# soldasim/BOSS.jl

Hardware: AMD Instinct MI355X
Metric: gp_posterior_updates_per_sec (+ acq_evals_per_sec), N=4096 d=8 fp64 (higher is better)
Workload: dtype f64; 1 GPU; d=8 synthetic blackbox, GaussianProcess(Matern52) surrogate, N=4096 fp64 posterior update + ExpectedImprovement over 8192 candidates per GPU (BASELINE.json configs[1]+[2]); N=4096, d=8, M_per_gpu=8192, kernel=matern52, parallelism=single GPU: no exchange

## Files before the change

### boss.jl_amd/csrc/bosship.hip

```cpp
#include "../../include/bosship.h"

#include <hip/hip_runtime.h>

#include <algorithm>
#include <cmath>
#include <cstdint>
#include <cstdio>
#include <cstdlib>
#include <atomic>
#include <chrono>
#include <cstring>
#include <functional>
#include <limits>
#include <map>
#include <mutex>
#include <string>
#include <thread>
#include <vector>

#include "gp_kernels.hpp"
#include "potrf.hpp"
#include "chain.hpp"
#include "small_calls.hpp"
#include "rider.hpp"
// ... 42 lines not shown
}

constexpr size_t MULTI_RES_OFF = 384;
constexpr size_t FEW_RES_OFF = 400;

struct Workspace {
    void* p = nullptr;
    size_t bytes = 0;
};

struct Ctx {
    int device = -1;
    int logical = -1;
    hipStream_t own_stream = nullptr;
    hipStream_t stream = nullptr;
    hipStream_t side_stream = nullptr;
    std::vector<hipEvent_t> ev_panel, ev_rest;
    hipEvent_t ev_fork = nullptr, ev_up = nullptr;
    unsigned long long* sig_panel = nullptr;
    unsigned long long* sig_panel_host = nullptr;
    unsigned long long sig_seq = 0;
    hipStream_t chain_stream = nullptr, strip_stream = nullptr;
    unsigned long long chain_seq = 0, crit_seq = 0, up_seq = 0;
    int n_cus = 256;
    bool chain_ok = false;
    bool test_drop_chain = false;
    unsigned long long acq_seq = 0;
    unsigned long long few_seq = 0;
    std::mutex slab_mtx;
    void* slab_cache = nullptr;
    size_t slab_cache_bytes = 0;
    void* hostblk_cache = nullptr;
    size_t hostblk_cache_bytes = 0;
    unsigned long long* few_done = nullptr;
    unsigned long long few_done_cnt = 0;
    bool lookahead = true;
    bool prof_on = false;
    std::map<std::string, std::vector<std::pair<hipEvent_t, hipEvent_t>>> prof;
    std::vector<hipEvent_t> ev_pool;
    Workspace vscratch, csc, pred, acq, batchA, batchX, batchMisc, craw, lgA, lgB, lgC, few, setdesc, setmom;
    static constexpr int LLG_BANKS = 4;
    Workspace lgbank[LLG_BANKS - 1][3];
    hipStream_t llg_stream[LLG_BANKS - 1] = {nullptr, nullptr, nullptr};
    hipEvent_t llg_join[LLG_BANKS - 1] = {nullptr, nullptr, nullptr};
    void* pinned = nullptr;
    struct TrailTab {
        TrailWork* dev = nullptr;
        std::vector<TrailWork> host;
        std::vector<int> off;
    };
    TrailTab trail[65];
    std::mutex mtx;
};

static void chain_quiesce(Ctx* c) {
    if (c->chain_stream) (void)hipStreamSynchronize(c->chain_stream);
    if (c->strip_stream) (void)hipStreamSynchronize(c->strip_stream);
}

static std::mutex g_ctx_mtx;
static std::map<int, Ctx*> g_ctx;

static bool release_cached_slabs() {
    int dev = -1;
    if (hipGetDevice(&dev) != hipSuccess) return false;
    std::vector<void*> blocks;
// ... 5 lines not shown
            std::lock_guard<std::mutex> sl(c->slab_mtx);
            if (c->slab_cache) blocks.push_back(c->slab_cache);
            c->slab_cache = nullptr;
            c->slab_cache_bytes = 0;
        }
    }
    for (void* b : blocks) (void)hipFree(b);
    return !blocks.empty();
}
extern "C" int boss_debug_fail_next_alloc(int n) {
    g_fail_allocs.store(n > 0 ? n : 0);
    return BOSS_OK;
}
extern "C" int boss_debug_slab_cache_bytes(int device, size_t* bytes_out) {
    std::lock_guard<std::mutex> lk(g_ctx_mtx);
    auto it = g_ctx.find(device);
    if (bytes_out) *bytes_out = 0;
    if (it != g_ctx.end() && bytes_out) {
        std::lock_guard<std::mutex> sl(it->second->slab_mtx);
        *bytes_out = it->second->slab_cache_bytes;
    }
    return BOSS_OK;
}

static void ctx_destroy(Ctx* c) {
    if (!c) return;
    if (c->own_stream) (void)hipStreamDestroy(c->own_stream);
    if (c->side_stream) (void)hipStreamDestroy(c->side_stream);
    if (c->chain_stream) (void)hipStreamDestroy(c->chain_stream);
    if (c->strip_stream) (void)hipStreamDestroy(c->strip_stream);
    if (c->ev_fork) (void)hipEventDestroy(c->ev_fork);
    if (c->sig_panel && !c->sig_panel_host) (void)hipFree(c->sig_panel);
    if (c->few_done) (void)hipFree(c->few_done);
    for (auto& t : c->trail)
        if (t.dev) (void)hipFree(t.dev);
    if (c->slab_cache) (void)hipFree(c->slab_cache);
    if (c->hostblk_cache) (void)hipHostFree(c->hostblk_cache);
    if (c->ev_up) (void)hipEventDestroy(c->ev_up);
    for (int i = 0; i < Ctx::LLG_BANKS - 1; ++i) {
        if (c->llg_stream[i]) (void)hipStreamDestroy(c->llg_stream[i]);
        if (c->llg_join[i]) (void)hipEventDestroy(c->llg_join[i]);
    }
    if (c->pinned) (void)hipHostFree(c->pinned);
    delete c;
}

static int ctx_init(Ctx* c) {
    {
        int least = 0, greatest = 0;
        (void)hipDeviceGetStreamPriorityRange(&least, &greatest);
        static const int cu_mask = getenv("BOSS_CU_MASK") ? atoi(getenv("BOSS_CU_MASK")) : 0;
        if (cu_mask) {
            hipDeviceProp_t prop;
            HIPCHK(hipGetDeviceProperties(&prop, c->device));
            const int ncu = prop.multiProcessorCount, words = (ncu + 31) / 32;
            auto make = [&](hipStream_t* st, int lo, int hi) {
                std::vector<uint32_t> m(words, 0u);
                for (int b = lo; b < hi && b < ncu; ++b) m[b / 32] |= 1u << (b % 32);
                return hipExtStreamCreateWithCUMask(st, (uint32_t)words, m.data());
            };
            HIPCHK(make(&c->chain_stream, 0, 16));
            HIPCHK(make(&c->strip_stream, 16, 32));
            HIPCHK(make(&c->own_stream, 32, ncu));
            HIPCHK(make(&c->side_stream, cu_mask >= 2 ? 40 : 32, cu_mask >= 2 ? ncu : ncu - 8));
            c->stream = c->own_stream;
            std::fprintf(stderr, "[bosship] BOSS_CU_MASK=%d: chain on CU bits 0-15, strips on 16-31, main stream on 32-%d, side stream %d-%d\n",
// ... 241 lines not shown
    bool gated = false;
    bool chained = false;
    bool fell_back = false;
    int trail_used = -1;
    double* host_res = nullptr;
    double* host_res_dev = nullptr;
    bool par_in_args = false;
    unsigned long long res_seq = 0;
    bool res_polled = false;
    double* host_par = nullptr;
    hipEvent_t par_ev = nullptr;
    unsigned long long epoch = 0;
    unsigned long long factor_gen = 0, dinv0_gen = ~0ull;
    hipEvent_t dinv_ev = nullptr;
    bool dinv_pending = false;
    bool aug = false;
    int npts = 0, ldx = 0;
    bool gibbs = false;
    double *lamX = nullptr, *ampX = nullptr, *noiseX = nullptr;
    double *Winv = nullptr, *Linv = nullptr;
    double* W2 = nullptr;
    int w2_np = 0;
    unsigned long long w2_gen = ~0ull;
    bool w2_used = false;
    bool have_winv = false;
    int few_calls = 0;
    int append_calls = 0;
};

struct boss_cand {
    Ctx* ctx = nullptr;
    int d = 0, M = 0, Mp = 0;
    double* Craw = nullptr;
};

struct boss_track {
    Ctx* ctx = nullptr;
    boss_gp* gp = nullptr;
    int d = 0, M = 0, Mp = 0, tiles = 0, Ncap = 0, N = 0;
    unsigned long long epoch = 0;
    double *V = nullptr, *Csc = nullptr, *mu = nullptr, *var = nullptr, *mean = nullptr;
    bool has_mean = false;
};

static inline int round_up(int x, int m) { return (x + m - 1) / m * m; }
struct SetBatch {
    int nb = 1;
    size_t sA = 0, sInv16 = 0, sDinv = 0, sDinv2 = 0, sW = 0, sX = 0;
};
static void linv_enqueue(boss_gp* g, hipStream_t s, double* U, double* Lw, const SetBatch& B = SetBatch());
constexpr int MAX_ROWS = 46080;

extern "C" const char* boss_version(void) { return "bosship 0.1.0 (gfx950, fp64 MFMA)"; }
extern "C" const char* boss_last_error(void) { return g_last_error.c_str(); }

extern "C" int boss_device_count(int* n_out) {
    const int n = visible_devices();
    hipError_t e = n > 0 ? hipSuccess : hipErrorNoDevice;
    if (e != hipSuccess || n <= 0) {
        if (n_out) *n_out = 0;
        return fail(BOSS_E_NO_DEVICE, "no HIP device visible (bosship has no CPU fallback)");
    }
    if (n_out) *n_out = n;
    return BOSS_OK;
}

extern "C" int boss_set_stream(int device, void* hip_stream) {
    Ctx* c;
    int rc = get_ctx(device, &c);
    if (rc) return rc;
    std::lock_guard<std::mutex> lk(c->mtx);
    HIPCHK(hipStreamSynchronize(c->stream));
    c->stream = hip_stream ? (hipStream_t)hip_stream : c->own_stream;
    return BOSS_OK;
}

extern "C" int boss_device_sync(int device) {
    Ctx* c;
    int rc = get_ctx(device, &c);
    if (rc) return rc;
    HIPCHK(hipStreamSynchronize(c->stream));
    return BOSS_OK;
}

static bool few_done_ensure(Ctx* c, hipStream_t s) {
    if (c->few_done) return true;
    if (hipMalloc((void**)&c->few_done, sizeof(unsigned long long)) != hipSuccess) {
        (void)hipGetLastError();
        c->few_done = nullptr;
        return false;
    }
    (void)hipMemsetAsync(c->few_done, 0, sizeof(unsigned long long), s);
    c->few_done_cnt = 0;
    return true;
}
static bool few_fused() {
    static const bool v = !(getenv("BOSS_FEW_FUSED") && atoi(getenv("BOSS_FEW_FUSED")) == 0);
    return v;
}

#include "host_factor.inc"
#include "host_append.inc"
#include "host_batch.inc"
#include "host_predict.inc"
#include "host_acq.inc"
#include "host_rider.inc"
#include "host_track.inc"
#include "host_multi.inc"

extern "C" int boss_bench_mfma_f64(int device, int iters, double* tflops_out) {
    Ctx* c;
    int rc = get_ctx(device, &c);
    if (rc) return rc;
    hipDeviceProp_t prop;
    HIPCHK(hipGetDeviceProperties(&prop, device));
    const int blocks = prop.multiProcessorCount;
    double* sink;
    HIPCHK(dev_malloc((void**)&sink, 8));
    hipEvent_t e0, e1;
    HIPCHK(hipEventCreate(&e0));
    HIPCHK(hipEventCreate(&e1));
    hipLaunchKernelGGL(mfma_f64_rate_kernel, dim3(blocks), dim3(256), 0, c->stream, iters / 8 + 1, sink);
    HIPCHK(hipEventRecord(e0, c->stream));
    hipLaunchKernelGGL(mfma_f64_rate_kernel, dim3(blocks), dim3(256), 0, c->stream, iters, sink);
    HIPCHK(hipEventRecord(e1, c->stream));
    HIPCHK(hipEventSynchronize(e1));
    float ms = 0.f;
    HIPCHK(hipEventElapsedTime(&ms, e0, e1));
// ... 125 lines not shown
```

### boss.jl_amd/csrc/host_acq.inc

```

static int acq_ei_impl(int P, int S, boss_gp_t* const* gps, const boss_cand_t* cand, const double* mean_Xs,
                       const double* fit_coefs, const double* y_max, int has_best, double best,
                       const unsigned char* valid_mask, double* acq_out, long* argmax_out, double* max_out,
                       double* dpair, long idx_off, bool defer) {
    if (P < 1 || S < 1 || !gps || !cand || !fit_coefs) return fail(BOSS_E_INVALID, "bad arguments");
    Ctx* c = cand->ctx;
    HIPCHK(hipSetDevice(c->device));
    for (int i = 0; i < P * S; ++i) {
        if (!gps[i]) return fail(BOSS_E_INVALID, "NULL posterior handle");
        if (gps[i]->ctx != c) return fail(BOSS_E_INVALID, "all handles and candidates must live on one device");
        if (!gps[i]->fitted) return fail(BOSS_E_NOT_FITTED, "handle has no valid factorisation");
    }
    std::lock_guard<std::mutex> lk(c->mtx);
    hipStream_t s = c->stream;
    const int M = cand->M;
    const size_t nd = (size_t)3 * P * M + M + 2 * P;
    {
        int rc = ws_reserve(c->acq, sizeof(double) * nd + M);
        if (rc) return rc;
    }
    double* dev = (double*)c->acq.p;
    double* dmu = dev;
    double* dvar = dmu + (size_t)P * M;
    double* dacq = dvar + (size_t)P * M;
    double* dmean = dacq + M;
    double* dcoef = dmean + (size_t)P * M;
    double* dymax = dcoef + P;
    unsigned char* dmask = (unsigned char*)(dev + nd);
    double* hres = (double*)c->pinned + (defer ? MULTI_RES_OFF : 0);
    EiPar par;
    int rc = ei_params(c, s, P, fit_coefs, y_max, has_best, best, &par, dcoef, dymax);
    if (rc) return rc;
    if (valid_mask) (void)hipMemcpyAsync(dmask, valid_mask, M, hipMemcpyHostToDevice, s);
    if (S > 1) (void)hipMemsetAsync(dacq, 0, sizeof(double) * M, s);
    std::vector<double> hmean;
    static const bool set_off = getenv("BOSS_NO_SET_PREDICT") && atoi(getenv("BOSS_NO_SET_PREDICT"));
    if (S > 1 && par.mode != 0 && !set_off && predict_set_ok(P * S, gps, cand)) {
        const size_t pm = (size_t)P * M;
        rc = ws_reserve(c->setmom, sizeof(double) * pm * S * (mean_Xs ? 3 : 2));
        if (rc) return rc;
        double* mu_all = (double*)c->setmom.p;
        double* var_all = mu_all + pm * S;
        double* mean_all = mean_Xs ? var_all + pm * S : nullptr;
        if (mean_Xs) {
            hmean.resize(pm * S);
            for (int sm = 0; sm < S; ++sm)
                for (int j = 0; j < M; ++j)
                    for (int p = 0; p < P; ++p) hmean[pm * sm + (size_t)p * M + j] = mean_Xs[p + (size_t)P * (j + (size_t)M * sm)];
            (void)hipMemcpyAsync(mean_all, hmean.data(), sizeof(double) * pm * S, hipMemcpyHostToDevice, s);
            (void)hipStreamSynchronize(s);
        }
        rc = predict_set_enqueue(P * S, gps, cand, mean_all, mu_all, var_all, (size_t)M);
        if (rc) {
            (void)hipStreamSynchronize(s);
            return rc;
        }
        hipLaunchKernelGGL(ei_accumulate_set_kernel, dim3((M + 255) / 256), dim3(256), 0, s, (const double*)mu_all, (const double*)var_all, pm, M, M,
                           0, S - 1, par, dcoef, dymax, dacq);
        hipLaunchKernelGGL(acq_epilogue_kernel, dim3(1), dim3(ACQ_EPI_THREADS), 0, s, (const double*)(mu_all + pm * (S - 1)),
                           (const double*)(var_all + pm * (S - 1)), M, M, par, dcoef, dymax, dacq, 1, 1.0 / S, valid_mask ? dmask : nullptr, hres,
                           (acq_out || defer) ? 0ull : ++c->acq_seq, dpair, idx_off);
    } else
    for (int sm = 0; sm < S; ++sm) {
        if (par.mode != 0) {
            if (mean_Xs) {
                hmean.resize((size_t)P * M);
                for (int j = 0; j < M; ++j)
                    for (int p = 0; p < P; ++p) hmean[(size_t)p * M + j] = mean_Xs[p + (size_t)P * (j + (size_t)M * sm)];
                (void)hipMemcpyAsync(dmean, hmean.data(), sizeof(double) * P * M, hipMemcpyHostToDevice, s);
                (void)hipStreamSynchronize(s);
            }
            for (int p = 0; p < P; ++p) {
                rc = predict_enqueue(gps[p + (size_t)P * sm], cand, mean_Xs ? dmean + (size_t)p * M : nullptr,
                                     dmu + (size_t)p * M, dvar + (size_t)p * M);
                if (rc) {
                    (void)hipStreamSynchronize(s);
                    return rc;
                }
            }
        }
        ProfScope ps(c, sm + 1 < S ? "ei" : "argmax");
        if (sm + 1 < S)
            hipLaunchKernelGGL(ei_accumulate_kernel, dim3((M + 255) / 256), dim3(256), 0, s, dmu, dvar, M, M, par, dcoef, dymax,
                               dacq);
        else
            hipLaunchKernelGGL(acq_epilogue_kernel, dim3(1), dim3(ACQ_EPI_THREADS), 0, s, dmu, dvar, M, M, par, dcoef, dymax,
                               dacq, S > 1 ? 1 : 0, 1.0 / S, valid_mask ? dmask : nullptr, hres, (acq_out || defer) ? 0ull : ++c->acq_seq,
                               dpair, idx_off);
    }
    if (acq_out) (void)hipMemcpyAsync(acq_out, dacq, sizeof(double) * M, hipMemcpyDeviceToHost, s);
    if (defer) {
        hipError_t e0 = hipGetLastError();
        return e0 == hipSuccess ? BOSS_OK : fail(BOSS_E_NO_DEVICE, hipGetErrorString(e0));
    }
    bool got = false;
    if (!acq_out) {
        volatile unsigned long long* seq = reinterpret_cast<volatile unsigned long long*>(hres) + 2;
        for (unsigned long i = 1;; ++i) {
            if (*seq == c->acq_seq) {
                got = true;
                break;
            }
            if ((i & 0x3fff) == 0 && hipStreamQuery(s) != hipErrorNotReady) break;
        }
        std::atomic_thread_fence(std::memory_order_acquire);
    }
    hipError_t e = got ? hipSuccess : hipStreamSynchronize(s);
    hipError_t e2 = hipGetLastError();
    if (e != hipSuccess) return fail(BOSS_E_NO_DEVICE, hipGetErrorString(e));
    if (e2 != hipSuccess) return fail(BOSS_E_NO_DEVICE, hipGetErrorString(e2));
    if (argmax_out) std::memcpy(argmax_out, &hres[1], sizeof(long));
    if (max_out) *max_out = hres[0];
    return BOSS_OK;
}

extern "C" int boss_acq_ei(int P, int S, boss_gp_t* const* gps, const boss_cand_t* cand, const double* mean_Xs,
                           const double* fit_coefs, const double* y_max, int has_best, double best,
                           const unsigned char* valid_mask, double* acq_out, long* argmax_out, double* max_out) {
    return acq_ei_impl(P, S, gps, cand, mean_Xs, fit_coefs, y_max, has_best, best, valid_mask, acq_out, argmax_out, max_out, nullptr, 0, false);
}

// ... 214 lines not shown
```

### boss.jl_amd/csrc/host_append.inc

```

static int gp_own(boss_gp* g) {
    if (!g->set) return BOSS_OK;
    Ctx* c = g->ctx;
    hipStream_t s = c->stream;
    const size_t Np = g->Np, d = g->d;
    double* nw[10] = {nullptr, nullptr, nullptr, nullptr, nullptr, nullptr, nullptr, nullptr, nullptr, nullptr};
    double* src[10] = {g->Xraw, g->Xsc, g->y, g->mean, g->A, g->inv16, g->Dinv, g->Dinv2, g->invlam, g->scal};
    const size_t bytes[10] = {sizeof(double) * d * Np, sizeof(double) * d * Np, sizeof(double) * Np, sizeof(double) * Np,
                              sizeof(double) * (size_t)g->ld * Np, sizeof(double) * g->nblk * 8 * 256, sizeof(double) * g->nblk * BLK * BLK,
                              sizeof(double) * Np * PRED_RB, sizeof(double) * (d + 4), sizeof(double) * 4};
    double *hres = nullptr, *hpar = nullptr, *hres_dev = nullptr;
    bool ok = true;
    for (int i = 0; i < 10 && ok; ++i) ok = dev_malloc((void**)&nw[i], bytes[i]) == hipSuccess;
    ok = ok && hipHostMalloc((void**)&hres, 512, hipHostMallocDefault) == hipSuccess &&
         hipHostMalloc((void**)&hpar, sizeof(double) * (d + 4), hipHostMallocDefault) == hipSuccess &&
         hipHostGetDevicePointer((void**)&hres_dev, hres, 0) == hipSuccess;
    dinv_join(g);
    hipError_t e = hipSuccess;
    for (int i = 0; i < 10 && ok && e == hipSuccess; ++i) e = hipMemcpyAsync(nw[i], src[i], bytes[i], hipMemcpyDeviceToDevice, s);
    if (ok && e == hipSuccess) e = hipStreamSynchronize(s);
    if (!ok || e != hipSuccess) {
        (void)hipStreamSynchronize(s);
        (void)hipGetLastError();
        for (double* p : nw)
// ... 160 lines not shown
    if (rc) return rc;
    g->fitted = false;
    g->have_lt = false;
    ++g->factor_gen;
    if (!fast) {
        g->have_dinv = false;
        g->have_winv = false;
        g->few_calls = 0;
    }
    static const bool args_off = getenv("BOSS_NO_FEW_ARGS") && atoi(getenv("BOSS_NO_FEW_ARGS"));
    const bool by_args = fast && n == 1 && d <= FEW_ARGS_MAX_D && !args_off;
    if (!by_args) {
        std::vector<double> xb;
        pack_points(xb, X_new, d, n, n, g->discrete.empty() ? nullptr : g->discrete.data());
        HIPCHK(hipMemcpy2DAsync(g->Xraw + N0, sizeof(double) * g->Np, xb.data(), sizeof(double) * n, sizeof(double) * n, d,
                                hipMemcpyHostToDevice, s));
        HIPCHK(hipMemcpyAsync(g->y + N0, y_new, sizeof(double) * n, hipMemcpyHostToDevice, s));
        if (mean_new) {
            HIPCHK(hipMemcpyAsync(g->mean + N0, mean_new, sizeof(double) * n, hipMemcpyHostToDevice, s));
            g->has_mean = true;
        }
        HIPCHK(hipStreamSynchronize(s));
    }
    g->N = N1;
    if (fast) {
        const int Np = g->Np, ld = g->ld, nwg = Np / WINV_ROWS;
        dinv_join(g);
        if (!g->have_dinv) {
            dinv_launch(g, s);
            g->have_dinv = true;
        }
        rc = ws_reserve(c->few, sizeof(double) * ((size_t)Np * 32 + (size_t)nwg * 8 + 2 * (size_t)Np + 8));
        if (rc) return rc;
        rc = ws_reserve(c->csc, sizeof(double) * (size_t)d * 64);
        if (rc) return rc;
        double* R = (double*)c->few.p;
        double* part = R + (size_t)Np * 32;
        double* lvec = part + (size_t)nwg * 8;
        double* wvec = lvec + Np;
        double* dz = wvec + Np;
        double* Csc = (double*)c->csc.p;
        bool fused_done = false;
        if (by_args) {
            AppendPoint ap;
            FewCand fc;
            ap.d = d;
            ap.N0 = N0;
            ap.Np = Np;
            ap.y = y_new[0];
            ap.mean = mean_new ? mean_new[0] : 0.0;
            fc.ncols = 1;
            for (int j = 0; j < WINV_MAX_M; ++j) {
                fc.mean[j] = 0.0;
                for (int k = 0; k < FEW_ARGS_MAX_D; ++k) fc.x[j][k] = 0.0;
            }
            for (int k = 0; k < FEW_ARGS_MAX_D; ++k) {
                double v = k < d ? X_new[k] : 0.0;
                if (k < d && !g->discrete.empty() && g->discrete[k]) v = std::nearbyint(v);
                ap.raw[k] = v;
                ap.sc[k] = k < d ? v * g->host_par[k] : 0.0;
                fc.x[0][k] = ap.sc[k];
            }
            if (mean_new) g->has_mean = true;
            const bool fused = few_fused() && few_done_ensure(c, s) && sizeof(double) * (size_t)Np <= 144 * 1024;
            if (fused) {
                hipLaunchKernelGGL(kstar_args_kernel, dim3(Np / 256), dim3(256), 0, s, fc, (const double*)g->Xsc, Np, N0, d, g->kernel, g->amp2, R, 1);
// ... 144 lines not shown
```

### boss.jl_amd/csrc/host_predict.inc

```

extern "C" int boss_cand_create(int device, int d, int M, const double* Xs, boss_cand_t** out) {
    if (!out) return fail(BOSS_E_INVALID, "out is NULL");
    *out = nullptr;
    if (d < 1 || M < 1 || !Xs) return fail(BOSS_E_INVALID, "need d >= 1, M >= 1 and non-NULL Xs");
    Ctx* c;
    int rc = get_ctx(device, &c);
    if (rc) return rc;
    boss_cand* cd = new boss_cand();
    cd->ctx = c;
    cd->d = d;
    cd->M = M;
    cd->Mp = round_up(M, 64);
    if (dev_malloc((void**)&cd->Craw, sizeof(double) * d * cd->Mp) != hipSuccess) {
        delete cd;
        return fail(BOSS_E_ALLOC, "device allocation failed");
    }
    std::vector<double> buf;
    pack_points(buf, Xs, d, M, cd->Mp, nullptr);
    HIPCHK(hipMemcpy(cd->Craw, buf.data(), sizeof(double) * d * cd->Mp, hipMemcpyHostToDevice));
    *out = cd;
    return BOSS_OK;
}

static int drain(Ctx* c, int rc) {
    (void)hipStreamSynchronize(c->stream);
    return rc;
}

static int neg_var_error(long* bad_index, unsigned long long bad, double v) {
    if (bad_index) *bad_index = (long)bad;
    char msg[160];
    std::snprintf(msg, sizeof msg, "The posterior GP predicted variance %g but only values above -1e-08 are tolerated. (DomainError)", v);
    return fail(BOSS_E_NEG_VAR, msg);
}

struct DownCopy {
    void* host;
    const void* dev;
    size_t bytes;
};
static int finish(Ctx* c, std::initializer_list<DownCopy> outs) {
    hipStream_t s = c->stream;
    const char* next = (const char*)outs.begin()->dev;
    size_t total = 0;
    bool together = true;
// ... 81 lines not shown
    const int Np = g->Np, ld = g->ld;
    hipLaunchKernelGGL(linv_seed_kernel, dim3(PRED_RB, Np / PRED_RB, B.nb), dim3(PRED_RB), 0, s, (const double*)g->Dinv2, Lw, ld, U, ld,
                       B.sDinv2, B.sW);
    for (int sz = PRED_RB; sz < Np; sz *= 2) {
        const int pairs = (Np + 2 * sz - 1) / (2 * sz), tiles = (sz / BLK) * (sz / BLK);
        hipLaunchKernelGGL((linv_level_kernel<SyrkG, 1>), dim3(tiles, pairs, B.nb), dim3(256), 0, s, (const double*)g->A, ld, Lw, ld, U, ld,
                           Np, sz, B.sA, B.sW);
        hipLaunchKernelGGL((linv_level_kernel<SyrkG, 2>), dim3(tiles, pairs, B.nb), dim3(256), 0, s, (const double*)g->A, ld, Lw, ld, U, ld,
                           Np, sz, B.sA, B.sW);
    }
}

static void gibbs_kstar32_launch(boss_gp* g, const boss_cand* cd, const double* clam_dev, const double* camp_dev, int tiles,
                                 double* out, hipStream_t s) {
    if (g->d <= GIBBS_KSTAR_MAX_D)
        hipLaunchKernelGGL(gibbs_kstar_cols_kernel, dim3(g->Np / 256, tiles), dim3(256),
                           sizeof(double) * (2 * g->d * 32 + 32 + 2 * 8 * 256), s, (const double*)g->Xraw, (const double*)g->lamX,
                           (const double*)g->ampX, g->d, g->N, g->Np, (const double*)cd->Craw, clam_dev, camp_dev, cd->Mp, out);
    else
        hipLaunchKernelGGL(gibbs_kstar_kernel<32>, dim3(g->Np / 256, tiles), dim3(256), sizeof(double) * (2 * g->d + 1) * 32, s,
                           (const double*)g->Xraw, (const double*)g->lamX, (const double*)g->ampX, g->d, g->N, g->Np,
                           (const double*)cd->Craw, clam_dev, camp_dev, cd->Mp, out);
}

static void small_dinv(boss_gp* g, hipStream_t s) {
    dinv_join(g);
    if (g->have_dinv || g->dinv0_gen == g->factor_gen) return;
    hipLaunchKernelGGL(potrf_dinv_kernel, dim3(8, 1, 1), dim3(64), 0, s, g->A, g->ld, (size_t)0, g->inv16, (size_t)0, g->Dinv, (size_t)0);
    g->dinv0_gen = g->factor_gen;
}
static bool small_predict_ok(const boss_gp* g, int M) {
    const long long cap = std::min<long long>(16384, 1024LL * SMALL_MAX_N * SMALL_MAX_N / ((long long)g->N * g->N));
    return small_fit_ok(g->ctx, g->N, g->d) && M <= cap && !g->aug && !g->gibbs;
}

static int predict_enqueue(boss_gp* g, const boss_cand* cd, const double* mean_s_dev, double* mu, double* var,
                           bool for_grad = false, const double* clam_dev = nullptr, const double* camp_dev = nullptr,
                           bool need_v = false) {
    Ctx* c = g->ctx;
    hipStream_t s = c->stream;
    if (!g->fitted) return fail(BOSS_E_NOT_FITTED, "handle has no valid factorisation");
    if (g->gibbs && !clam_dev)
        return fail(BOSS_E_INVALID, "nonstationary posteriors predict through boss_ngp_predict (λ(x*), α(x*) are needed)");
    if (cd->ctx != c) return fail(BOSS_E_INVALID, "candidates and posterior live on different devices");
    if (cd->d != g->d) return fail(BOSS_E_INVALID, "candidate dimension differs from the model's x_dim");
    if (!for_grad && !need_v && small_predict_ok(g, cd->M)) {
        small_dinv(g, s);
        const int grid = std::min(512, (cd->M + SPG_WAVES - 1) / SPG_WAVES);
        hipLaunchKernelGGL(small_predict_grad_kernel<false>, dim3(grid), dim3(SPG_THREADS), SPG_LDS_BYTES, s, (const double*)g->Dinv,
                           (const double*)g->A, g->ld, g->Np, g->N, g->d, g->kernel, g->amp2, (const double*)g->Xsc, g->ldx,
                           (const double*)cd->Craw, cd->Mp, cd->M, (const double*)g->invlam, (const unsigned char*)g->discrete_dev,
                           mean_s_dev, (const double*)nullptr, mu, var, (double*)nullptr, (double*)nullptr);
        HIPCHK(hipGetLastError());
        return BOSS_OK;
    }
    bool joined = false;
    auto join_dinv = [&]() {
        if (!joined) dinv_join(g);
        joined = true;
    };
    if (!g->have_dinv) {
        join_dinv();
        ProfScope ps(c, "dinv");
        dinv_launch(g, s);
        g->have_dinv = true;
    }
    g->dinv_used = true;
    const int Mp = cd->Mp;
    const int BN = slab_bn(cd->M, for_grad);
    const int tiles = (cd->M + BN - 1) / BN;
    int rc = ws_reserve(c->csc, sizeof(double) * (size_t)g->d * Mp);
    if (rc) return rc;
    rc = ws_reserve(c->vscratch, sizeof(double) * (size_t)tiles * BN * g->Np * (for_grad ? 2 : 1));
    if (rc) return rc;
    double* Csc = (double*)c->csc.p;
    if (!g->gibbs)
        hipLaunchKernelGGL(scale_cand_kernel, dim3((Mp + 255) / 256), dim3(256), 0, s, cd->Craw, Csc, g->invlam,
                           g->discrete_dev, g->d, Mp);
#ifdef BOSS_EXPERIMENTS
    static const int dbg = getenv("BOSS_DBG") ? atoi(getenv("BOSS_DBG")) : 0;
#else
    constexpr int dbg = 0;
#endif
    static const bool no_few = getenv("BOSS_NO_FEW") && atoi(getenv("BOSS_NO_FEW"));
    static const int few_max_tiles = getenv("BOSS_FEW_MAX_TILES") ? atoi(getenv("BOSS_FEW_MAX_TILES")) : 128;
    const int ftiles = (cd->M + 31) / 32;
    const size_t aug_lds = sizeof(double) * ((size_t)g->d * (64 + 256) + g->d);
    if (ftiles <= few_max_tiles && g->Np >= 4 * PRED_RB && g->d <= 64 && !no_few && (BN == 32 || for_grad)) {
        typedef PredG32 G;
        typedef GemmDirect<4, 1, 2, 2, 8> GU;
        ProfScope ps(c, "predict");
        const int nb = g->Np / PRED_RB;
        const int nwg = g->Np / WINV_ROWS;
        const size_t step_part = (size_t)ftiles * nb * FEW_STEP_PARTS * 64;
        rc = ws_reserve(c->few, sizeof(double) * ((size_t)ftiles * ((size_t)g->Np * 32 + 64) + (size_t)nwg * 8 + step_part));
        if (rc) return rc;
        double* R = (double*)c->few.p;
        double* ssmz = R + (size_t)ftiles * g->Np * 32;
        double* part = ssmz + 64 * (size_t)ftiles + (size_t)nwg * 8;
        double* V = (double*)c->vscratch.p;
        static const int winv_after = getenv("BOSS_WINV_AFTER") ? atoi(getenv("BOSS_WINV_AFTER")) : 2;
        const size_t winv_lds = sizeof(double) * (size_t)g->Np * (cd->M == 1 ? 1 : cd->M == 2 ? 2 : WINV_MAX_M);
        if (winv_after > 0 && !g->have_winv && ++g->few_calls >= winv_after) {
            const size_t bytes = sizeof(double) * (size_t)g->ld * g->Np;
            bool ok = (g->Winv != nullptr || dev_malloc((void**)&g->Winv, bytes) == hipSuccess) &&
                      (g->Linv != nullptr || dev_malloc((void**)&g->Linv, bytes) == hipSuccess);
            if (ok) {
                join_dinv();
                linv_enqueue(g, s, g->Winv, g->Linv);
// ... 177 lines not shown
            const boss_gp* g = gps[i];
            uniform = g->set == g0->set && !g->have_dinv && !g->dinv_pending && g->A - g0->A == sA * i && g->inv16 - g0->inv16 == sI * i &&
                      g->Dinv - g0->Dinv == sD * i && g->Dinv2 - g0->Dinv2 == sD2 * i && sA > 0 && sI > 0 && sD > 0 && sD2 > 0;
        }
        if (uniform) {
            SetBatch B;
            B.nb = n;
            B.sA = (size_t)sA;
            B.sInv16 = (size_t)sI;
            B.sDinv = (size_t)sD;
            B.sDinv2 = (size_t)sD2;
            dinv_launch(gps[0], s, B);
            for (int i = 0; i < n; ++i) gps[i]->have_dinv = true;
        }
        for (int i = 0; i < n; ++i) {
            boss_gp* g = gps[i];
            dinv_join(g);
            if (!g->have_dinv) {
                dinv_launch(g, s);
                g->have_dinv = true;
            }
            g->dinv_used = true;
        }
    }
    static const size_t v_cap = (size_t)(getenv("BOSS_SET_V_GIB") ? atof(getenv("BOSS_SET_V_GIB")) : 8.0) * ((size_t)1 << 30);
    const size_t v_one = sizeof(double) * (size_t)tiles * G::BN * Np;
    int group = (int)std::max<size_t>(1, std::min<size_t>((size_t)n, std::min<size_t>(v_cap / v_one, 65535)));
    int rc = ws_reserve(c->vscratch, v_one * group);
    while (rc == BOSS_E_ALLOC && group > 1) {
        group = (group + 1) / 2;
        rc = ws_reserve(c->vscratch, v_one * group);
    }
    if (rc) return rc;
    rc = ws_reserve(c->csc, sizeof(double) * (size_t)d * Mp * n);
    if (rc) return rc;
    rc = ws_reserve(c->setdesc, sizeof(PredSet) * (size_t)n);
    if (rc) return rc;
    std::vector<PredSet> desc(n);
    for (int i = 0; i < n; ++i) {
        const boss_gp* g = gps[i];
        desc[i].A = g->A;
        desc[i].Dinv = g->Dinv2;
        desc[i].Xsc = g->Xsc;
        desc[i].Csc = (const double*)c->csc.p + (size_t)i * d * Mp;
        desc[i].mean_s = mean_all ? mean_all + (size_t)i * mstride : nullptr;
        desc[i].invlam = g->invlam;
        desc[i].mu = mu_all + (size_t)i * mstride;
        desc[i].var = var_all + (size_t)i * mstride;
        desc[i].amp2 = g->amp2;
    }
    const size_t bytes = sizeof(PredSet) * (size_t)n;
    if (bytes <= PINNED_UP_BYTES) {
        void* stage = (char*)c->pinned + PINNED_UP_OFF;
        HIPCHK(hipEventSynchronize(c->ev_up));
        std::memcpy(stage, desc.data(), bytes);
        HIPCHK(hipMemcpyAsync(c->setdesc.p, stage, bytes, hipMemcpyHostToDevice, s));
        HIPCHK(hipEventRecord(c->ev_up, s));
    } else {
        HIPCHK(hipMemcpyAsync(c->setdesc.p, desc.data(), bytes, hipMemcpyHostToDevice, s));
        HIPCHK(hipStreamSynchronize(s));
    }
    const PredSet* dsets = (const PredSet*)c->setdesc.p;
    for (int i0 = 0; i0 < n; i0 += 65535)
        hipLaunchKernelGGL(scale_cand_set_kernel, dim3((Mp + 255) / 256, std::min(65535, n - i0)), dim3(256), 0, s, (const double*)cd->Craw,
                           dsets + i0, (const unsigned char*)g0->discrete_dev, d, Mp);
    for (int i0 = 0; i0 < n; i0 += group) {
// ... 631 lines not shown
```

### boss.jl_amd/csrc/host_rider.inc

```

static int rider_max_m() {
    static const int v = getenv("BOSS_RIDER_MAX_M") ? std::min(8192, atoi(getenv("BOSS_RIDER_MAX_M"))) : 4096;
    return v;
}
static bool rider_off() {
    static const bool v = getenv("BOSS_NO_RIDER") && atoi(getenv("BOSS_NO_RIDER"));
    return v;
}
static int rider_chunks(int nstrips) {
    static const int env = getenv("BOSS_RIDER_CHUNKS") ? atoi(getenv("BOSS_RIDER_CHUNKS")) : 0;
    if (env > 0) return std::min(env, RIDER_MAX_CH);
    static const int max_wgs = getenv("BOSS_RIDER_MAX_WGS") ? atoi(getenv("BOSS_RIDER_MAX_WGS")) : 240;
    const int fit = (max_wgs - nstrips) / nstrips;
    if (fit >= 4) return std::min(RIDER_MAX_CH, fit);
    return nstrips <= 64 ? 6 : 4;
}

struct RiderRun {
    boss_gp* g = nullptr;
    const boss_cand* cd = nullptr;
    double *Csc = nullptr, *V = nullptr, *part = nullptr, *part_ss = nullptr, *part_z = nullptr, *pairs = nullptr;
    size_t part_n = 0;
    int nstrips = 0, nch = 1, slots = 0;
    const ChainPlan* plan = nullptr;
    bool interleaved = false;
    bool s_only = false;
};
static int rider_reserve(RiderRun& r) {
    Ctx* c = r.g->ctx;
    const int Np = r.g->Np, nblk = r.g->nblk, Mp = r.cd->Mp;
    r.nstrips = Mp / 32;
    r.nch = rider_chunks(r.nstrips);
    int rc = ws_reserve(c->csc, sizeof(double) * (size_t)r.g->d * Mp);
    if (rc) return rc;
    rc = ws_reserve(c->vscratch, sizeof(double) * (size_t)r.nstrips * 32 * Np);
    if (rc) return rc;
    const size_t part_n = (size_t)RIDER_MAX_CH * r.nstrips * BLK * 32, blk_n = (size_t)nblk * Mp;
    rc = ws_reserve(c->few, sizeof(double) * (2 * part_n + 2 * blk_n + 2 * (size_t)r.nstrips));
    if (rc) return rc;
    r.Csc = (double*)c->csc.p;
    r.V = (double*)c->vscratch.p;
    r.part = (double*)c->few.p;
    r.part_n = part_n;
    r.part_ss = r.part + 2 * part_n;
    r.part_z = r.part_ss + blk_n;
    r.pairs = r.part_z + blk_n;
    if (!few_done_ensure(c, c->stream)) return fail(BOSS_E_ALLOC, "device allocation failed");
    return BOSS_OK;
}
static void rider_step(RiderRun& r, int k) {
    boss_gp* g = r.g;
    Ctx* c = g->ctx;
    hipStream_t s = c->side_stream;
    const int nblk = g->nblk, Mp = r.cd->Mp;
    const unsigned long long base = r.plan->cbase;
    const unsigned budget = poll_budget_ticks(g->Np);
    if (k == 0) {
        hipLaunchKernelGGL(rider_gate_kernel, dim3(1), dim3(64), 0, s, (const unsigned long long*)(c->sig_panel + SIGW_WDONE), 1, 1, base + 1,
                           g->info, budget, 500);
        hipLaunchKernelGGL(scale_cand_kernel, dim3((Mp + 255) / 256), dim3(256), 0, s, r.cd->Craw, r.Csc, g->invlam, g->discrete_dev, g->d, Mp);
    }
    RiderStep p;
    p.A = g->A;
    p.inv16 = g->inv16;
    p.V = r.V;
// ... 241 lines not shown
```

### boss.jl_amd/csrc/small_calls.hpp

```cpp
#pragma once
#include "potrf.hpp"

namespace boss {

struct AppendTail {
    double y, mean;
    int N0;
    const double* hyp;
    double *scal, *dz, *vout;
    int* info;
};
template <int MC, bool APPEND = false>
__global__ __launch_bounds__(256) void winv_args_kernel(FewCand par, const double* __restrict__ Xsc, int N, int d, int kern, double amp2,
                                                        const double* __restrict__ U, int ldu, int Np,
                                                        const double* __restrict__ Afac, int ld, const double* __restrict__ kst,
                                                        double* __restrict__ part,
                                                        unsigned long long* __restrict__ done, unsigned long long done_after,
                                                        double* __restrict__ host_out, unsigned long long seq, AppendTail tail = AppendTail()) {
    extern __shared__ double ks[];
    const int tid = threadIdx.x, lane = tid & 63, wave = tid >> 6;
    const int kb = (gridDim.x - 1 - blockIdx.x) * WINV_ROWS;
    constexpr int KU = 8;
    const int cend = kb + WINV_ROWS;
    if (kst) {
    } else
    for (int c0 = tid; c0 < cend; c0 += 256 * KU) {
        double r2[KU][MC];
#pragma unroll
        for (int u = 0; u < KU; ++u)
#pragma unroll
            for (int j = 0; j < MC; ++j) r2[u][j] = 0.0;
        for (int kd = 0; kd < d; ++kd) {
            double xr[KU];
#pragma unroll
// ... 81 lines not shown
        if constexpr (APPEND) {
            const double d2 = tail.hyp[0] + tail.hyp[1] - red[0];
            const int inf = (d2 > 0.0) ? 0 : tail.N0 + 1;
            *tail.info = inf;
            const double dd = sqrt(d2), zn = (tail.y - tail.mean - red[256]) / dd;
            tail.dz[0] = dd;
            tail.dz[1] = zn;
            tail.scal[0] += 2.0 * log(dd);
            tail.scal[1] = __builtin_fma(zn, zn, tail.scal[1]);
            host_out[0] = tail.scal[0];
            host_out[1] = tail.scal[1];
            reinterpret_cast<int*>(host_out + 2)[0] = inf;
            __threadfence_system();
            __hip_atomic_store(reinterpret_cast<unsigned long long*>(host_out + 3), seq, __ATOMIC_RELAXED, __HIP_MEMORY_SCOPE_SYSTEM);
            return;
        }
        long long bad = -1;
        for (int j = 0; j < M; ++j) {
            const double s = red[(2 * j) * 256], z = red[(2 * j + 1) * 256];
            double v = amp2 - s + PREDICT_JITTER;
            if (!(v >= 0.0)) {
                if (v >= -MAX_NEG_VAR) v = 0.0;
                else if (bad < 0) bad = j;
            }
            host_out[j] = par.mean[j] + z;
            host_out[4 + j] = v;
        }
        reinterpret_cast<long long*>(host_out)[8] = bad;
        __threadfence_system();
        __hip_atomic_store(reinterpret_cast<unsigned long long*>(host_out) + 9, seq, __ATOMIC_RELAXED, __HIP_MEMORY_SCOPE_SYSTEM);
    }
}

}
```

Baseline: 884.2 updates/s.

## Parallelize acquisition epilogue across workgroups and reuse scaled candidate matrix

Replaces the single-workgroup EI epilogue with a multi-workgroup kernel. Each block computes EI values and a local argmax, and the last block to finish, detected through an atomic counter, merges the partial results. Separately, it caches a key (candidate id, inverse lengthscales, discrete mask, buffer pointer) so the candidate scaling kernel is skipped when the scaled candidates are already current. The cache adds host-side invalidation points that must be kept correct, and the cross-call reuse could be a staleness risk if the key misses a change.

Measured after the change: 889.4 updates/s, median of 2. Within noise of the previous version (+0.6%).

```diff
diff --git a/boss.jl_amd/csrc/bosship.hip b/boss.jl_amd/csrc/bosship.hip
--- a/boss.jl_amd/csrc/bosship.hip
+++ b/boss.jl_amd/csrc/bosship.hip
@@ -98,6 +98,16 @@
     size_t slab_cache_bytes = 0;
     void* hostblk_cache = nullptr;
     size_t hostblk_cache_bytes = 0;
+    struct CscKey {
+        unsigned long long cand_id = 0;
+        const void* p = nullptr;
+        size_t bytes = 0;
+        int d = 0, Mp = 0;
+        std::vector<double> invlam;
+        std::vector<unsigned char> discrete;
+    } csc_key;
+    double* epi_part = nullptr;
+    unsigned long long* epi_done = nullptr;
     unsigned long long* few_done = nullptr;
     unsigned long long few_done_cnt = 0;
     bool lookahead = true;
@@ -169,6 +179,7 @@
     if (c->ev_fork) (void)hipEventDestroy(c->ev_fork);
     if (c->sig_panel && !c->sig_panel_host) (void)hipFree(c->sig_panel);
     if (c->few_done) (void)hipFree(c->few_done);
+    if (c->epi_part) (void)hipFree(c->epi_part);
     for (auto& t : c->trail)
         if (t.dev) (void)hipFree(t.dev);
     if (c->slab_cache) (void)hipFree(c->slab_cache);
@@ -476,6 +487,7 @@
     Ctx* ctx = nullptr;
     int d = 0, M = 0, Mp = 0;
     double* Craw = nullptr;
+    unsigned long long id = 0;
 };
 
 struct boss_track {
@@ -538,6 +550,21 @@
     c->few_done_cnt = 0;
     return true;
 }
+static bool epi_mwg_ensure(Ctx* c, hipStream_t s) {
+    static const bool off = getenv("BOSS_ACQ_EPI_MWG") && atoi(getenv("BOSS_ACQ_EPI_MWG")) == 0;
+    if (off) return false;
+    if (c->epi_part) return true;
+    const size_t bytes = sizeof(double) * 2 * ACQ_MWG_MAX_WG + 128;
+    if (hipMalloc((void**)&c->epi_part, bytes) != hipSuccess) {
+        (void)hipGetLastError();
+        c->epi_part = nullptr;
+        return false;
+    }
+    (void)hipMemsetAsync(c->epi_part, 0, bytes, s);
+    c->epi_done = reinterpret_cast<unsigned long long*>(c->epi_part + 2 * ACQ_MWG_MAX_WG + 8);
+    return true;
+}
+static void csc_forget(Ctx* c) { c->csc_key.cand_id = 0; }
 static bool few_fused() {
     static const bool v = !(getenv("BOSS_FEW_FUSED") && atoi(getenv("BOSS_FEW_FUSED")) == 0);
     return v;
diff --git a/boss.jl_amd/csrc/host_acq.inc b/boss.jl_amd/csrc/host_acq.inc
--- a/boss.jl_amd/csrc/host_acq.inc
+++ b/boss.jl_amd/csrc/host_acq.inc
@@ -1,3 +1,16 @@
+
+static void acq_epilogue_launch(Ctx* c, hipStream_t s, const double* mu, const double* var, int M, const EiPar& par, const double* dcoef,
+                                const double* dymax, double* dacq, int have_prev, double inv_s, const unsigned char* dmask, double* hres,
+                                unsigned long long seq, double* dpair, long idx_off) {
+    if (epi_mwg_ensure(c, s)) {
+        const int grid = std::min(ACQ_MWG_MAX_WG, (M + ACQ_MWG_THREADS - 1) / ACQ_MWG_THREADS);
+        hipLaunchKernelGGL(acq_epilogue_mwg_kernel, dim3(grid), dim3(ACQ_MWG_THREADS), 0, s, mu, var, M, M, par, dcoef, dymax, dacq, have_prev,
+                           inv_s, dmask, hres, seq, dpair, idx_off, c->epi_part, c->epi_done);
+    } else {
+        hipLaunchKernelGGL(acq_epilogue_kernel, dim3(1), dim3(ACQ_EPI_THREADS), 0, s, mu, var, M, M, par, dcoef, dymax, dacq, have_prev, inv_s,
+                           dmask, hres, seq, dpair, idx_off);
+    }
+}
 
 static int acq_ei_impl(int P, int S, boss_gp_t* const* gps, const boss_cand_t* cand, const double* mean_Xs,
                        const double* fit_coefs, const double* y_max, int has_best, double best,
@@ -57,9 +70,8 @@
         }
         hipLaunchKernelGGL(ei_accumulate_set_kernel, dim3((M + 255) / 256), dim3(256), 0, s, (const double*)mu_all, (const double*)var_all, pm, M, M,
                            0, S - 1, par, dcoef, dymax, dacq);
-        hipLaunchKernelGGL(acq_epilogue_kernel, dim3(1), dim3(ACQ_EPI_THREADS), 0, s, (const double*)(mu_all + pm * (S - 1)),
-                           (const double*)(var_all + pm * (S - 1)), M, M, par, dcoef, dymax, dacq, 1, 1.0 / S, valid_mask ? dmask : nullptr, hres,
-                           (acq_out || defer) ? 0ull : ++c->acq_seq, dpair, idx_off);
+        acq_epilogue_launch(c, s, (const double*)(mu_all + pm * (S - 1)), (const double*)(var_all + pm * (S - 1)), M, par, dcoef, dymax, dacq, 1,
+                            1.0 / S, valid_mask ? dmask : nullptr, hres, (acq_out || defer) ? 0ull : ++c->acq_seq, dpair, idx_off);
     } else
     for (int sm = 0; sm < S; ++sm) {
         if (par.mode != 0) {
@@ -84,9 +96,8 @@
             hipLaunchKernelGGL(ei_accumulate_kernel, dim3((M + 255) / 256), dim3(256), 0, s, dmu, dvar, M, M, par, dcoef, dymax,
                                dacq);
         else
-            hipLaunchKernelGGL(acq_epilogue_kernel, dim3(1), dim3(ACQ_EPI_THREADS), 0, s, dmu, dvar, M, M, par, dcoef, dymax,
-                               dacq, S > 1 ? 1 : 0, 1.0 / S, valid_mask ? dmask : nullptr, hres, (acq_out || defer) ? 0ull : ++c->acq_seq,
-                               dpair, idx_off);
+            acq_epilogue_launch(c, s, dmu, dvar, M, par, dcoef, dymax, dacq, S > 1 ? 1 : 0, 1.0 / S, valid_mask ? dmask : nullptr, hres,
+                                (acq_out || defer) ? 0ull : ++c->acq_seq, dpair, idx_off);
     }
     if (acq_out) (void)hipMemcpyAsync(acq_out, dacq, sizeof(double) * M, hipMemcpyDeviceToHost, s);
     if (defer) {
diff --git a/boss.jl_amd/csrc/host_append.inc b/boss.jl_amd/csrc/host_append.inc
--- a/boss.jl_amd/csrc/host_append.inc
+++ b/boss.jl_amd/csrc/host_append.inc
@@ -216,6 +216,7 @@
         }
         rc = ws_reserve(c->few, sizeof(double) * ((size_t)Np * 32 + (size_t)nwg * 8 + 2 * (size_t)Np + 8));
         if (rc) return rc;
+        csc_forget(c);
         rc = ws_reserve(c->csc, sizeof(double) * (size_t)d * 64);
         if (rc) return rc;
         double* R = (double*)c->few.p;
diff --git a/boss.jl_amd/csrc/host_predict.inc b/boss.jl_amd/csrc/host_predict.inc
--- a/boss.jl_amd/csrc/host_predict.inc
+++ b/boss.jl_amd/csrc/host_predict.inc
@@ -11,6 +11,8 @@
     cd->d = d;
     cd->M = M;
     cd->Mp = round_up(M, 64);
+    static std::atomic<unsigned long long> next_id{0};
+    cd->id = ++next_id;
     if (dev_malloc((void**)&cd->Craw, sizeof(double) * d * cd->Mp) != hipSuccess) {
         delete cd;
         return fail(BOSS_E_ALLOC, "device allocation failed");
@@ -158,6 +160,27 @@
 static bool small_predict_ok(const boss_gp* g, int M) {
     const long long cap = std::min<long long>(16384, 1024LL * SMALL_MAX_N * SMALL_MAX_N / ((long long)g->N * g->N));
     return small_fit_ok(g->ctx, g->N, g->d) && M <= cap && !g->aug && !g->gibbs;
+}
+
+static bool csc_current(Ctx* c, const boss_gp* g, const boss_cand* cd) {
+    static const bool off = getenv("BOSS_CSC_REUSE") && atoi(getenv("BOSS_CSC_REUSE")) == 0;
+    Ctx::CscKey& k = c->csc_key;
+    if (off || !cd->id || g->aug || !g->host_par) {
+        k.cand_id = 0;
+        return false;
+    }
+    const int d = g->d;
+    const bool same = k.cand_id == cd->id && k.p == c->csc.p && k.bytes == c->csc.bytes && k.d == d && k.Mp == cd->Mp &&
+                      k.discrete == g->discrete && std::memcmp(k.invlam.data(), g->host_par, sizeof(double) * d) == 0;
+    if (same) return true;
+    k.cand_id = cd->id;
+    k.p = c->csc.p;
+    k.bytes = c->csc.bytes;
+    k.d = d;
+    k.Mp = cd->Mp;
+    k.discrete = g->discrete;
+    k.invlam.assign(g->host_par, g->host_par + d);
+    return false;
 }
 
 static int predict_enqueue(boss_gp* g, const boss_cand* cd, const double* mean_s_dev, double* mu, double* var,
@@ -200,7 +223,7 @@
     rc = ws_reserve(c->vscratch, sizeof(double) * (size_t)tiles * BN * g->Np * (for_grad ? 2 : 1));
     if (rc) return rc;
     double* Csc = (double*)c->csc.p;
-    if (!g->gibbs)
+    if (!g->gibbs && !csc_current(c, g, cd))
         hipLaunchKernelGGL(scale_cand_kernel, dim3((Mp + 255) / 256), dim3(256), 0, s, cd->Craw, Csc, g->invlam,
                            g->discrete_dev, g->d, Mp);
 #ifdef BOSS_EXPERIMENTS
@@ -444,6 +467,7 @@
         rc = ws_reserve(c->vscratch, v_one * group);
     }
     if (rc) return rc;
+    csc_forget(c);
     rc = ws_reserve(c->csc, sizeof(double) * (size_t)d * Mp * n);
     if (rc) return rc;
     rc = ws_reserve(c->setdesc, sizeof(PredSet) * (size_t)n);
diff --git a/boss.jl_amd/csrc/host_rider.inc b/boss.jl_amd/csrc/host_rider.inc
--- a/boss.jl_amd/csrc/host_rider.inc
+++ b/boss.jl_amd/csrc/host_rider.inc
@@ -31,6 +31,7 @@
     const int Np = r.g->Np, nblk = r.g->nblk, Mp = r.cd->Mp;
     r.nstrips = Mp / 32;
     r.nch = rider_chunks(r.nstrips);
+    csc_forget(c);
     int rc = ws_reserve(c->csc, sizeof(double) * (size_t)r.g->d * Mp);
     if (rc) return rc;
     rc = ws_reserve(c->vscratch, sizeof(double) * (size_t)r.nstrips * 32 * Np);
diff --git a/boss.jl_amd/csrc/small_calls.hpp b/boss.jl_amd/csrc/small_calls.hpp
--- a/boss.jl_amd/csrc/small_calls.hpp
+++ b/boss.jl_amd/csrc/small_calls.hpp
@@ -1,5 +1,6 @@
 #pragma once
 #include "potrf.hpp"
+#include "acq_kernels.hpp"
 
 namespace boss {
 
@@ -147,4 +148,83 @@
     }
 }
 
-}
+constexpr int ACQ_MWG_THREADS = 256, ACQ_MWG_MAX_WG = 256;
+constexpr long ACQ_NONE = 0x7fffffffffffffffL;
+__device__ __forceinline__ void argmax_merge(double& bv, long& bi, double ov, long oi) {
+    if (oi != ACQ_NONE && (bi == ACQ_NONE || better(ov, oi, bv, bi))) {
+        bv = ov;
+        bi = oi;
+    }
+}
+__device__ __forceinline__ void argmax_workgroup(double& bv, long& bi, double* sv, long* si) {
+#pragma unroll
+    for (int off = 32; off >= 1; off >>= 1) {
+        const double ov = __shfl_xor(bv, off);
+        const long oi = (long)__shfl_xor((long long)bi, off);
+        argmax_merge(bv, bi, ov, oi);
+    }
+    const int lane = threadIdx.x & 63, wave = threadIdx.x >> 6;
+    if (lane == 0) {
+        sv[wave] = bv;
+        si[wave] = bi;
+    }
+    __syncthreads();
+    if (threadIdx.x == 0)
+        for (int w = 1; w < ACQ_MWG_THREADS / 64; ++w) argmax_merge(bv, bi, sv[w], si[w]);
+}
+__global__ __launch_bounds__(ACQ_MWG_THREADS) void acq_epilogue_mwg_kernel(const double* __restrict__ mu, const double* __restrict__ var,
+                                                                           int ldm, int M, EiPar par,
+                                                                           const double* __restrict__ coefs_dev,
+                                                                           const double* __restrict__ ymax_dev,
+                                                                           double* __restrict__ acq_sum, int have_prev, double inv_s,
+                                                                           const unsigned char* __restrict__ mask,
+                                                                           double* __restrict__ res, unsigned long long res_seq,
+                                                                           double* __restrict__ dpair, long idx_off,
+                                                                           double* __restrict__ part, unsigned long long* __restrict__ done) {
+    __shared__ double sv[ACQ_MWG_THREADS / 64];
+    __shared__ long si[ACQ_MWG_THREADS / 64];
+    __shared__ int lastflag;
+    double bv = -INFINITY;
+    long bi = ACQ_NONE;
+    for (int j = blockIdx.x * ACQ_MWG_THREADS + threadIdx.x; j < M; j += gridDim.x * ACQ_MWG_THREADS) {
+        double a = ei_value(mu, var, ldm, j, par, coefs_dev, ymax_dev);
+        if (have_prev) a += acq_sum[j];
+        a *= inv_s;
+        if (mask && !mask[j]) a = 0.0;
+        acq_sum[j] = a;
+        argmax_merge(bv, bi, a, j);
+    }
+    argmax_workgroup(bv, bi, sv, si);
+    if (threadIdx.x == 0) {
+        st_sc1(part + 2 * blockIdx.x, bv);
+        st_sc1(part + 2 * blockIdx.x + 1, __longlong_as_double((long long)bi));
+        drain_stores();
+        const unsigned long long before = __hip_atomic_fetch_add(as_global(done), 1ull, __ATOMIC_RELAXED, __HIP_MEMORY_SCOPE_AGENT);
+        lastflag = (before + 1 == gridDim.x) ? 1 : 0;
+    }
+    __syncthreads();
+    if (lastflag == 0) return;
+    __syncthreads();
+    bv = -INFINITY;
+    bi = ACQ_NONE;
+    if (threadIdx.x < gridDim.x) {
+        bv = ld_sc1(part + 2 * threadIdx.x);
+        bi = (long)__double_as_longlong(ld_sc1(part + 2 * threadIdx.x + 1));
+    }
+    argmax_workgroup(bv, bi, sv, si);
+    if (threadIdx.x == 0) {
+        raise_word(done, 0ull);
+        if (dpair) {
+            dpair[0] = bv;
+            dpair[1] = (double)(bi + idx_off);
+        }
+        res[0] = bv;
+        reinterpret_cast<long*>(res)[1] = bi;
+        if (res_seq) {
+            __threadfence_system();
+            __hip_atomic_store(reinterpret_cast<unsigned long long*>(res) + 2, res_seq, __ATOMIC_RELAXED, __HIP_MEMORY_SCOPE_SYSTEM);
+        }
+    }
+}
+
+}
```
